# zdebruine/singlet

Measured on AMD Instinct MI355X. Metric: ALS iterations/sec (1M cells x 30k genes, 5% nnz, k=50), higher is better.
Workload: dtype f64

## Files before the change

### singlet_amd/csrc/kernels_dense.hip

```cpp
#include "sgl_internal.h"

typedef double d4 __attribute__((ext_vector_type(4)));

template <int NT>
__global__ __launch_bounds__(256) void gram_mfma_kernel(const double* __restrict__ F, int k, int64_t cols,
                                                        int64_t cols_per_block, double* __restrict__ part) {
    constexpr int NTILES = NT * (NT + 1) / 2;
    const int lane = threadIdx.x & 63, wave = threadIdx.x >> 6;
    const int r16 = lane & 15, kk = lane >> 4;
    const int64_t c_begin = (int64_t)blockIdx.x * cols_per_block;
    int64_t c_end = c_begin + cols_per_block;
    if (c_end > cols) c_end = cols;

    d4 acc[NTILES];
#pragma unroll
    for (int t = 0; t < NTILES; ++t) acc[t] = d4{0, 0, 0, 0};

    for (int64_t c = c_begin + 4 * wave; c < c_end; c += 16) {
        const int64_t cc = c + kk;
        double f[NT];
#pragma unroll
        for (int b = 0; b < NT; ++b) {
            const int row = b * 16 + r16;
            f[b] = (cc < c_end && row < k) ? F[cc * k + row] : 0.0;
        }
        int t = 0;
#pragma unroll
        for (int bi = 0; bi < NT; ++bi)
#pragma unroll
            for (int bj = 0; bj <= bi; ++bj) {
                acc[t] = __builtin_amdgcn_mfma_f64_16x16x4f64(f[bi], f[bj], acc[t], 0, 0, 0);
                ++t;
            }
    }

    __shared__ double sm[4][64 * 4];
    double* out = part + (size_t)blockIdx.x * k * k;
    int t = 0;
#pragma unroll
    for (int bi = 0; bi < NT; ++bi)
#pragma unroll
        for (int bj = 0; bj <= bi; ++bj) {
            __syncthreads();
#pragma unroll
            for (int r = 0; r < 4; ++r) sm[wave][lane * 4 + r] = acc[t][r];
            __syncthreads();
            if (wave == 0) {
#pragma unroll
                for (int r = 0; r < 4; ++r) {
                    const double v = ((sm[0][lane * 4 + r] + sm[1][lane * 4 + r]) + sm[2][lane * 4 + r]) + sm[3][lane * 4 + r];
                    const int row = bi * 16 + kk + 4 * r;
                    const int col = bj * 16 + r16;
                    if (row < k && col < k) {
                        out[(size_t)col * k + row] = v;
                        if (bi != bj) out[(size_t)row * k + col] = v;
                    }
                }
// ... 153 lines not shown
        for (int q = 0; q < nseg; ++q) s += tmp[q * n + t];
        out[t] = s + add_all;
    }
}
static size_t sgl_partial_ws(int nblocks, int n) { return (size_t)nblocks * n + (size_t)((nblocks + SGL_RED_SEG - 1) / SGL_RED_SEG) * n; }
static int sgl_partial_sum(sgl_ctx* c, int nblocks, int n, int diag_k, double diag_add, double* out, double add_all = 0.0) {
    const int nseg = (nblocks + SGL_RED_SEG - 1) / SGL_RED_SEG;
    if (diag_k == 0 && n * nseg <= 1024) {
        partial_sum_small_kernel<<<dim3(1), dim3(1024), 0, c->stream>>>(c->ws, nblocks, n, nseg, add_all, out);
        HIPCHK(hipGetLastError());
        return SGL_OK;
    }
    if (add_all != 0.0) { sgl_set_error("partial sum: add_all only in the short form"); return SGL_EINVAL; }
    double* tmp = c->ws + (size_t)nblocks * n;
    partial_sum_stage1_kernel<<<dim3((n + 255) / 256, nseg), dim3(256), 0, c->stream>>>(c->ws, nblocks, n, tmp);
    HIPCHK(hipGetLastError());
    partial_sum_stage2_kernel<<<dim3((n + 255) / 256), dim3(256), 0, c->stream>>>(tmp, nseg, n, diag_k, diag_add, out);
    HIPCHK(hipGetLastError());
    return SGL_OK;
}

int k_gram_big_partials(hipStream_t s, const double* F, int k, int64_t cols, int64_t cols_per_block, int nblocks, double* part);

int k_gram(sgl_ctx* c, const double* F, int k, int64_t cols, double* G, double diag_add) {
    if (k <= 0 || k > SGL_MAX_K) { sgl_set_error("k_gram: k=%d out of range", k); return SGL_EINVAL; }
    int nblocks = (int)((cols + 255) / 256);
    if (nblocks > 1024) nblocks = 1024;
    const bool big_mfma = k > 128 && k <= 256 && !getenv("SGL_GRAM_BIG_VALU");
    if (k > 128 && nblocks > (big_mfma ? 512 : 128)) nblocks = big_mfma ? 512 : 128;
    if (nblocks < 1) nblocks = 1;
    int64_t cpb = (cols + nblocks - 1) / nblocks;
    cpb = (cpb + 15) / 16 * 16;
    nblocks = (int)((cols + cpb - 1) / cpb);
    if (nblocks < 1) nblocks = 1;
    SGLCHK(sgl_ws_reserve(c, sizeof(double) * sgl_partial_ws(nblocks, k * k)));
    hipStream_t s = c->stream;
    const int NT = (k + 15) / 16;
    if (NT == 1) gram_mfma_kernel<1><<<dim3(nblocks), dim3(256), 0, s>>>(F, k, cols, cpb, c->ws);
    else if (NT == 2) gram_mfma_kernel<2><<<dim3(nblocks), dim3(256), 0, s>>>(F, k, cols, cpb, c->ws);
    else if (NT == 3) gram_mfma_kernel<3><<<dim3(nblocks), dim3(256), 0, s>>>(F, k, cols, cpb, c->ws);
    else if (NT == 4) gram_mfma_kernel<4><<<dim3(nblocks), dim3(256), 0, s>>>(F, k, cols, cpb, c->ws);
    else if (NT == 5) gram_mfma_split_kernel<5><<<dim3(nblocks), dim3(256), 0, s>>>(F, k, cols, cpb, c->ws);
    else if (NT == 6) gram_mfma_split_kernel<6><<<dim3(nblocks), dim3(256), 0, s>>>(F, k, cols, cpb, c->ws);
    else if (NT == 7) gram_mfma_split_kernel<7><<<dim3(nblocks), dim3(256), 0, s>>>(F, k, cols, cpb, c->ws);
    else if (NT == 8) gram_mfma_split_kernel<8><<<dim3(nblocks), dim3(256), 0, s>>>(F, k, cols, cpb, c->ws);
    else if (big_mfma) SGLCHK(k_gram_big_partials(s, F, k, cols, cpb, nblocks, c->ws));
    else {
        const size_t lds = sizeof(double) * 16 * (size_t)k;
        if (lds > 48 * 1024) HIPCHK(hipFuncSetAttribute(reinterpret_cast<const void*>(&gram_valu_kernel), hipFuncAttributeMaxDynamicSharedMemorySize, 144 * 1024));
        for (int pair0 = 0; pair0 < k * k; pair0 += 256 * GV_MAXP)
            gram_valu_kernel<<<dim3(nblocks), dim3(256), lds, s>>>(F, k, cols, cpb, c->ws, pair0);
    }
    HIPCHK(hipGetLastError());
    return sgl_partial_sum(c, nblocks, k * k, k, diag_add, G);
}

__global__ void add_diag_kernel(double* __restrict__ G, int k, double v) {
    const int i = blockIdx.x * blockDim.x + threadIdx.x;
    if (i < k) G[(size_t)i * k + i] += v;
}

int k_gram_add_diag(hipStream_t s, double* G, int k, double v) {
    add_diag_kernel<<<dim3((k + 63) / 64), dim3(64), 0, s>>>(G, k, v);
    HIPCHK(hipGetLastError());
    return SGL_OK;
}

__global__ __launch_bounds__(256) void rowsum_kernel(const double* __restrict__ F, int k, int64_t cols,
                                                     int64_t cols_per_block, double* __restrict__ part) {
    const int tx = threadIdx.x & 63, ty = threadIdx.x >> 6;
    const int64_t c_begin = (int64_t)blockIdx.x * cols_per_block;
    int64_t c_end = c_begin + cols_per_block;
    if (c_end > cols) c_end = cols;
    __shared__ double sm[4][64];
    for (int r0 = 0; r0 < k; r0 += 64) {
        const int row = r0 + tx;
        double s0 = 0.0, s1 = 0.0;
        if (row < k) {
            int64_t cc = c_begin + ty;
            for (; cc + 28 < c_end; cc += 32) {
                double v[8];
#pragma unroll
                for (int u = 0; u < 8; ++u) v[u] = F[(cc + 4 * u) * k + row];
#pragma unroll
                for (int u = 0; u < 8; u += 2) { s0 += v[u]; s1 += v[u + 1]; }
            }
            for (; cc + 4 < c_end; cc += 8) {
                s0 += F[cc * k + row];
                s1 += F[(cc + 4) * k + row];
            }
            if (cc < c_end) s0 += F[cc * k + row];
        }
        __syncthreads();
        sm[ty][tx] = s0 + s1;
        __syncthreads();
        if (ty == 0 && row < k) part[(size_t)blockIdx.x * k + row] = ((sm[0][tx] + sm[1][tx]) + sm[2][tx]) + sm[3][tx];
    }
}


int k_rowsum(sgl_ctx* c, const double* F, int k, int64_t cols, double* d_out, int add_eps) {
    int nblocks = (int)((cols + 511) / 512);
// ... 4 lines not shown
    rowsum_kernel<<<dim3(nblocks), dim3(256), 0, c->stream>>>(F, k, cols, cpb, c->ws);
    HIPCHK(hipGetLastError());
    const int nseg = (nblocks + SGL_RED_SEG - 1) / SGL_RED_SEG;
    if (add_eps && k * nseg > 1024) { sgl_set_error("k_rowsum: add_eps needs the short form"); return SGL_EINVAL; }
    return sgl_partial_sum(c, nblocks, k, 0, 0.0, d_out, add_eps ? 1e-15 : 0.0);
}
bool k_rowsum_can_add_eps(int k, int64_t cols) {
    int nblocks = (int)((cols + 511) / 512);
    if (nblocks > 512) nblocks = 512;
    if (nblocks < 1) nblocks = 1;
    return k * ((nblocks + SGL_RED_SEG - 1) / SGL_RED_SEG) <= 1024;
}

__global__ void add_eps_kernel(double* __restrict__ d, int k) {
    const int i = blockIdx.x * blockDim.x + threadIdx.x;
    if (i < k) d[i] += 1e-15;
}

__global__ void scale_kernel(double* __restrict__ F, int k, int64_t n, const double* __restrict__ d) {
    for (int64_t t = (int64_t)blockIdx.x * blockDim.x + threadIdx.x; t < n; t += (int64_t)gridDim.x * blockDim.x)
        F[t] = F[t] / d[t % k];
}

int k_scale_apply(hipStream_t s, double* F, int k, int64_t cols, double* d, int add_eps) {
    if (add_eps) {
        add_eps_kernel<<<dim3((k + 63) / 64), dim3(64), 0, s>>>(d, k);
        HIPCHK(hipGetLastError());
    }
    const int64_t n = (int64_t)k * cols;
    if (n <= 0) return SGL_OK;
    int64_t blocks = (n + 255) / 256;
    if (blocks > 4096) blocks = 4096;
    scale_kernel<<<dim3((unsigned)blocks), dim3(256), 0, s>>>(F, k, n, d);
    HIPCHK(hipGetLastError());
    return SGL_OK;
}

__global__ __launch_bounds__(256) void cor_partial_kernel(const double* __restrict__ x, const double* __restrict__ y,
                                                          int64_t n, double* __restrict__ part) {
    double s[5] = {0, 0, 0, 0, 0};
    for (int64_t t = (int64_t)blockIdx.x * blockDim.x + threadIdx.x; t < n; t += (int64_t)gridDim.x * blockDim.x) {
        const double a = x[t], b = y[t];
        s[0] += a;
        s[1] += b;
        s[2] = fma(a, b, s[2]);
        s[3] = fma(a, a, s[3]);
        s[4] = fma(b, b, s[4]);
    }
    __shared__ double sm[5][256];
    for (int q = 0; q < 5; ++q) sm[q][threadIdx.x] = s[q];
    __syncthreads();
// ... 123 lines not shown
```

### singlet_amd/csrc/multi.hip

```cpp
#include "sgl_internal.h"

#include <dlfcn.h>
#include <rccl/rccl.h>
#include <string.h>
#include <stdlib.h>
#include <algorithm>
#include <atomic>
#include <chrono>
#include <condition_variable>
#include <memory>
#include <functional>
#include <mutex>
#include <string>
#include <thread>
#include <vector>

struct RcclApi {
    void* handle = nullptr;
    char path[512] = "";
    ncclResult_t (*GetUniqueId)(ncclUniqueId*) = nullptr;
    ncclResult_t (*CommInitRank)(ncclComm_t*, int, ncclUniqueId, int) = nullptr;
    ncclResult_t (*CommInitAll)(ncclComm_t*, int, const int*) = nullptr;
    ncclResult_t (*CommDestroy)(ncclComm_t) = nullptr;
    ncclResult_t (*CommAbort)(ncclComm_t) = nullptr;
// ... 589 lines not shown
    auto halo_solve = [&](int i) -> int {
        sgl_ctx* c = T->local[i];
        SGLCHK(sgl_step_h_solve(c, L1_h, L2_h, true));
        Phase ph(c, SGL_PH_RHS_W);
        return k_graph_pack(c->stream, c->graph, c->H, k, T->rank[i]);
    };
    auto halo_partials = [&](int i) -> int {
        sgl_ctx* c = T->local[i];
        { Phase ph(c, SGL_PH_RHS_W); SGLCHK(k_graph_conv(c->stream, c->graph, c->H, c->B, k)); }
        SGLCHK(partials(c, c->B));
        book(i);
        return SGL_OK;
    };
    auto exchange1 = [&](int who) -> int {
        return team_exchange(T, who, {{1, &red, (int64_t)k * mb, false}, {0, &tail, (int64_t)k * k + k, false}});
    };
    auto gene_block = [&](int i) -> int {
        sgl_ctx* c = T->local[i];
        const int r = T->rank[i];
        double* Gh = c->red + (size_t)k * mpad;
        double* sh = Gh + (size_t)k * k;
        { Phase ph(c, SGL_PH_SCALE);
          HIPCHK(hipMemcpyAsync(c->d, sh, sizeof(double) * k, hipMemcpyDeviceToDevice, c->stream));
          SGLCHK(k_scale_apply(c->stream, c->H, k, c->A.ncol, c->d, 1)); }
        const int64_t g0 = (int64_t)r * mb;
        const int64_t ng = std::max<int64_t>(0, std::min<int64_t>(mb, m - g0));
        { Phase ph(c, SGL_PH_GRAM);
          HIPCHK(hipMemcpyAsync(c->G, Gh, sizeof(double) * k * k, hipMemcpyDeviceToDevice, c->stream));
          SGLCHK(k_gram_rescale(c->stream, c->G, k, c->d, 1e-15)); }
        Phase ph(c, SGL_PH_NNLS_W);
        if (ng > 0) {
            double* Bblk = c->red + (size_t)g0 * k;
            SGLCHK(k_scale_apply(c->stream, Bblk, k, ng, c->d, 0));
            if (c->link_w) SGLCHK(k_link_mul(c->stream, Bblk, c->link_w + (size_t)g0 * c->link_w_rows, k, c->link_w_rows, ng));
            else if (c->glink_w.table) SGLCHK(k_link_mul_grouped(c->stream, Bblk, c->glink_w.table, c->glink_w.group + g0, k, c->glink_w.rows, c->glink_w.groups, ng));
            const int64_t* gene_nnz = (N > 1) ? c->col_nnz_At_global : c->col_nnz_At;
            if (N > 1 && !c->gene_nnz_global) { sgl_set_error("team: global gene counts missing"); return SGL_ESTATE; }
            SGLCHK(sgl_nnls_shared(c, c->G, Bblk, c->W + (size_t)g0 * k, (c->solve_empty || graph) ? nullptr : gene_nnz + g0, ng, L1_w, L2_w, c->sweep_counters + 1));
        }
        return SGL_OK;
    };
    auto exchange2 = [&](int who) -> int {
        if (N <= 1) return SGL_OK;
        return team_exchange(T, who, {{2, &wbuf, (int64_t)k * mb, false}});
    };
    auto tail_part = [&](int i) -> int { return sgl_scale_w_enqueue(T->local[i]); };
// ... 35 lines not shown
    const int N = T->nranks;
    const int k = T->local[0]->k;
    const int64_t m = T->nrow;
    const int64_t mb = N > 1 ? (m + N - 1) / N : m;
    const int64_t mpad = mb * N;
    std::vector<void*> dv(nl), red(nl), sb(nl), tail(nl), wbuf(nl);
    std::vector<double> tols(nl, 0.0);
    auto h_update = [&](int i) -> int {
        sgl_ctx* c = T->local[i];
        SGLCHK(sgl_step_begin(c));
        SGLCHK(sgl_predict_mask_dev(c, c->A, c->col_nnz_A, c->W, c->H, c->B, seed, inv_density, L1, L2, 0, SGL_PH_RHS_H,
                                    SGL_PH_NNLS_H, c->sweep_counters + 0));
        Phase ph(c, SGL_PH_SCALE);
        SGLCHK(k_rowsum(c, c->H, k, c->A.ncol, c->d));
        dv[i] = c->d;
        return SGL_OK;
    };
    auto exchange_d = [&](int who) -> int {
        if (N <= 1) return SGL_OK;
        return team_exchange(T, who, {{0, &dv, (int64_t)k, false}});
    };
    auto w_partials = [&](int i) -> int {
        sgl_ctx* c = T->local[i];
        { Phase ph(c, SGL_PH_SCALE); SGLCHK(k_scale_apply(c->stream, c->H, k, c->A.ncol, c->d, 1)); }
        if (N == 1) {
            const int64_t* gene_nnz = c->col_nnz_At;
            return sgl_predict_mask_dev(c, c->At, gene_nnz, c->H, c->W, c->red, seed, inv_density, L1, L2, 1, SGL_PH_RHS_W,
                                        SGL_PH_NNLS_W, c->sweep_counters + 1);
        }
        double* Bw = c->red;
        double* Gh = c->red + (size_t)k * mpad;
        { Phase ph(c, SGL_PH_GRAM); SGLCHK(k_gram(c, c->H, k, c->A.ncol, Gh, 0.0)); }
        { Phase ph(c, SGL_PH_RHS_W); SGLCHK(sgl_masked_rhs(c, 1, c->H, Bw, seed, inv_density)); }
        { Phase ph(c, SGL_PH_MASK);
          HIPCHK(hipMemsetAsync(c->Sbuf, 0, sizeof(double) * (size_t)mpad * k * k, c->stream));
          if (!c->gene_nnz_global) { sgl_set_error("team: global gene counts missing"); return SGL_ESTATE; }
          const DevMaskList* ML = nullptr;
          if (k <= 128 && !getenv("SGL_MASK_NO_LIST")) {
              SGLCHK(sgl_mask_list_select(c, 1, m, c->At.nrow, seed, inv_density, 1, 0, c->cell_offset));
              if (c->ML[1].mask_t == 1) ML = &c->ML[1];
          }
          SGLCHK(k_mask_gram_cols(c->stream, 0, m, c->At.nrow, c->col_nnz_At_global, c->H, nullptr, k, seed, inv_density, 1, 0,
                                  c->cell_offset, c->Sbuf, ML)); }
        red[i] = Bw;
        if (c->Stri) {
            Phase ph(c, SGL_PH_MASK);
// ... 530 lines not shown
```

### singlet_amd/csrc/sgl_internal.h

```cpp
#pragma once
#include <hip/hip_runtime.h>
#include <stdint.h>
#include <stdio.h>
#include <stdarg.h>
#include <atomic>
#include <functional>
#include <vector>
#include <algorithm>

#include "../../include/singlet_hip.h"

#define SGL_WAVE 64
#define SGL_MAX_K 1024
#define SGL_LANE_NNLS_MAX_K 128

void sgl_set_error(const char* fmt, ...);

hipError_t sgl_pool_malloc_raw(void** p, size_t bytes);
template <typename T_>
inline hipError_t sgl_pool_malloc(T_** p, size_t bytes) { return sgl_pool_malloc_raw(reinterpret_cast<void**>(p), bytes); }
hipError_t sgl_pool_free(void* p);
hipError_t sgl_pool_mem_info(size_t* free_b, size_t* total_b);
void sgl_pool_release(void);
size_t sgl_pool_cached_bytes(void);
// ... 143 lines not shown
    int32_t* group = nullptr;
    int rows = 0, groups = 0;
};

struct sgl_ctx {
    int device = 0;
    hipStream_t own_stream = nullptr;
    hipStream_t stream = nullptr;

    DevCSC A, At;
    DevTiled TA, TAt;
    bool use_tiled = false;
    int64_t cell_offset = 0, ncells_total = 0;
    int64_t* col_nnz_A = nullptr;
    int64_t* col_nnz_At = nullptr;
    int64_t* col_nnz_At_global = nullptr;
    bool gene_nnz_global = false;

    int k = 0;
    double *W = nullptr, *Wprev = nullptr, *H = nullptr, *d = nullptr;
    double* B = nullptr;
    double* red = nullptr;
    double* G = nullptr;
    double* Gpad = nullptr;
    NnlsScratch nnls_scr;
    bool solve_empty = false;
    double* Adense = nullptr;
    bool dense_gemm = false;
    void* rocblas = nullptr;
    double* link_h = nullptr;
    double* link_w = nullptr;
    int link_h_rows = 0, link_w_rows = 0;
    DevGroupLink glink_h, glink_w;
    DevGraph graph;
    bool dense_input = false;
    DevMaskList ML[2];
    int64_t ml_builds[2] = {0, 0};
    DevMaskList MLkeep[2][SGL_ML_KEEP];
    double* Gcols = nullptr;
    int64_t gcols_chunk = 0;
    double* Wd = nullptr;
    double* Sbuf = nullptr;
    double* Stri = nullptr;
    struct sgl_team* team = nullptr;
    int team_rank = 0;
    double* ws = nullptr;
    size_t ws_bytes = 0;
    double* scalars = nullptr;
    unsigned long long* sweep_counters = nullptr;
    int64_t sweeps_acc[4] = {0, 0, 0, 0};
    int64_t wave_sweeps_acc[2] = {0, 0};
    double* pinned = nullptr;
    int64_t knn_last[4] = {0, 0, 0, 0};
    int64_t markers_last[4] = {0, 0, 0, 0};
    int64_t gsea_last[5] = {0, 0, 0, 0, 0};

    sgl_allreduce_fn allreduce = nullptr;
    void* allreduce_user = nullptr;

    bool timing = false;
    std::vector<PhaseEvent> pending;
    std::vector<hipEvent_t> event_pool;
    double phase_ms[SGL_PH_COUNT] = {0};
    int64_t phase_calls[SGL_PH_COUNT] = {0};
};

int sgl_team_size(const sgl_ctx* c);
int sgl_nnls_shared(sgl_ctx* c, const double* G, double* B, double* X, const int64_t* col_nnz, int64_t ncols,
                    double L1, double L2, unsigned long long* counter, bool h_side = false);
int sgl_step_h_rhs(sgl_ctx* c, bool convolve);
int sgl_step_h_solve(sgl_ctx* c, double L1, double L2, bool convolve);
int sgl_graph_check(const char* who, const double* Gx, const int32_t* Gi, const int32_t* Gp, int32_t G_nrow, int32_t G_ncol, int64_t n);
int sgl_graph_upload(sgl_ctx* c, const char* who, const double* Gx, const int32_t* Gi, const int32_t* Gp, int32_t ncol);
void sgl_graph_clear(sgl_ctx* c);
inline bool sgl_has_links(const sgl_ctx* c) { return c->link_h || c->link_w || c->glink_h.table || c->glink_w.table; }
int sgl_scale_w_enqueue(sgl_ctx* c);
int sgl_scale_w_fetch(sgl_ctx* c, double* tol);
int sgl_mask_workspace(sgl_ctx* c);
int sgl_predict_mask_dev(sgl_ctx* c, const DevCSC& M, const int64_t* col_nnz, const double* F, double* X, double* Bbuf,
                         uint64_t seed, uint64_t inv_density, double L1, double L2, int mask_t, int rhs_phase, int nnls_phase,
                         unsigned long long* counter);
int sgl_mse_test_enqueue(sgl_ctx* c, uint64_t seed, uint64_t inv_density);
#define SGL_MASK_MAX_K SGL_MAX_K
void sgl_team_detach(sgl_ctx* c);

int sgl_phase_begin(sgl_ctx* c, int phase, PhaseEvent* pe);
int sgl_phase_end(sgl_ctx* c, PhaseEvent* pe);
int sgl_ws_reserve(sgl_ctx* c, size_t bytes);
// ... 59 lines not shown
                     const sgl_callbacks* cb);

int k_rand(hipStream_t s, uint64_t state, const uint64_t* i, const uint64_t* j, int64_t n, uint64_t* out);
int k_mask(hipStream_t s, uint64_t state, uint64_t inv_density, int64_t cell0, int32_t ncells, int32_t ngenes, uint8_t* out);
int k_synth_count(hipStream_t s, uint64_t S, uint64_t inv_density, int transposed, int64_t cell_offset,
                  int32_t ncells, int32_t ngenes, int64_t* counts, const double* skew_dev = nullptr);
int k_synth_fill(hipStream_t s, uint64_t S, uint64_t inv_density, const double* levels16_dev, int transposed,
                 int64_t cell_offset, int32_t ncells, int32_t ngenes, const int64_t* p, int32_t* idx, double* x,
                 const double* skew_dev = nullptr);
int k_synth_winit(hipStream_t s, uint64_t S, int k, int32_t ngenes, double* W);
int k_exclusive_scan(sgl_ctx* c, const int64_t* in, int64_t* out, int64_t n);
int k_scan_total(hipStream_t s, const int64_t* in, int64_t* out, int64_t n);
int k_col_counts(hipStream_t s, const int64_t* p, int64_t ncol, int64_t* counts);
int k_validate_csc(hipStream_t s, const int32_t* idx, const int64_t* p, int64_t ncol, int32_t nrow, int* flag_dev);
int k_all_finite(hipStream_t s, const double* x, int64_t n, int* flag_dev);
int k_widen_p(hipStream_t s, const int32_t* p32, int64_t n1, int64_t* p64);
int k_build_segments(hipStream_t s, const DevCSC& M);

int k_gram(sgl_ctx* c, const double* F, int k, int64_t cols, double* G, double diag_add);
int k_gram_add_diag(hipStream_t s, double* G, int k, double v);
int k_rowsum(sgl_ctx* c, const double* F, int k, int64_t cols, double* d_out, int add_eps = 0);
bool k_rowsum_can_add_eps(int k, int64_t cols);
int k_scale_apply(hipStream_t s, double* F, int k, int64_t cols, double* d, int add_eps);
int k_cor(sgl_ctx* c, const double* x, const double* y, int64_t n, double* out_dev);
int k_pad_gram(hipStream_t s, const double* G, int k, int KP, int GS, double* Gpad);
int k_gram_rescale(hipStream_t s, double* G, int k, const double* d, double diag_add);
int k_i64_to_f64(hipStream_t s, const int64_t* in, double* out, int64_t n);
int k_f64_to_i64(hipStream_t s, const double* in, int64_t* out, int64_t n);
int k_transpose_dense(hipStream_t s, const double* in, int rows, int cols, double* out);

int k_acc(hipStream_t s, const DevCSC& M, const double* F, int k, double* B,
          uint64_t mask_seed, uint64_t inv_density, int mask_mode, int64_t mask_col_offset, int64_t mask_row_offset);

void sgl_tiled_free(DevTiled& S);
int sgl_tiled_build(sgl_ctx* c, const DevCSC& M, int k, DevTiled& S);
int k_acc_tiled(hipStream_t s, const DevTiled& S, const double* F, int ldf, double* B, int ldb, int kf, const double* xvals = nullptr);
int k_acc_tiled_all(hipStream_t s, const DevTiled& S, const double* F, double* B, int k, const double* xvals = nullptr);
int sgl_tiled_mask_values(sgl_ctx* c, const DevCSC& M, DevTiled& S, uint64_t seed, uint64_t inv_density, int mask_t,
                          int64_t col_off, int64_t row_off);
int sgl_masked_rhs(sgl_ctx* c, int orientation, const double* F, double* Bbuf, uint64_t seed, uint64_t inv_density);
int tiled_part_size(int k);

int k_dense_count(hipStream_t s, const double* A, int32_t nrow, int64_t ncol, int64_t* counts);
int k_dense_fill(hipStream_t s, const double* A, int32_t nrow, int64_t ncol, const int64_t* p, int32_t* idx, double* x);
int k_dense_rhs(sgl_ctx* c, int which, const double* F, int k, double* B);
void sgl_dense_release(sgl_ctx* c);
// ... 159 lines not shown
```

### singlet_amd/csrc/singlet_hip.hip

```cpp
#include "sgl_internal.h"
#include "ingest_host.h"

#include <math.h>
#include <string.h>
#include <algorithm>
#include <string>
#include <chrono>
#include <mutex>
#include <vector>
#include <stdlib.h>

static thread_local char g_err[1024] = "";

void sgl_set_error(const char* fmt, ...) {
    va_list ap;
    va_start(ap, fmt);
    vsnprintf(g_err, sizeof(g_err), fmt, ap);
    va_end(ap);
}

extern "C" const char* sgl_last_error(void) { return g_err; }
extern "C" int sgl_abi_version(void) { return 2; }

struct CallTimes {
// ... 117 lines not shown
    g = DevGraph();
}
void sgl_graph_clear(sgl_ctx* c) { free_graph(c); }

static void links_clear(sgl_ctx* c) {
    dev_free(c->link_h);
    dev_free(c->link_w);
    c->link_h_rows = c->link_w_rows = 0;
    for (DevGroupLink* g : {&c->glink_h, &c->glink_w}) {
        dev_free(g->table);
        dev_free(g->group);
        *g = DevGroupLink();
    }
}

static void free_fit(sgl_ctx* c, bool keep_streams = false) {
    dev_free(c->W);
    dev_free(c->Wprev);
    dev_free(c->H);
    dev_free(c->d);
    dev_free(c->B);
    dev_free(c->red);
    dev_free(c->G);
    dev_free(c->Gpad);
    dev_free(c->Gcols);
    c->gcols_chunk = 0;
    dev_free(c->Wd);
    dev_free(c->Sbuf);
    dev_free(c->Stri);
    nnls_scratch_free(c->nnls_scr);
    links_clear(c);
    free_graph(c);
    dev_free(c->A.seg);
    dev_free(c->At.seg);
    if (!keep_streams) {
        sgl_tiled_free(c->TA);
        sgl_tiled_free(c->TAt);
        sgl_mask_lists_free_all(c);
    }
    c->use_tiled = false;
    c->k = 0;
}

static void free_matrix(sgl_ctx* c) {
    sgl_dense_release(c);
    free_csc(c->A);
// ... 764 lines not shown
    if (rc == SGL_OK) rc = sgl_weight_by_split(c, split_by, n_groups);
    if (rc == SGL_OK) rc = sgl_download_csc(c, 0, x_out, nullptr, nullptr);
    sgl_destroy(c);
    return rc;
}

static int64_t team_gene_block(const sgl_ctx* c) {
    const int64_t m = c->A.nrow;
    const int n = sgl_team_size(c);
    return n > 1 ? (m + n - 1) / n : m;
}

static int fit_init_impl(sgl_ctx* c, int32_t k, const double* w_init, uint64_t synth_seed) {
    const int64_t m = c->A.nrow, n = c->A.ncol;
    const int64_t mpad = team_gene_block(c) * std::max(1, sgl_team_size(c));
    sgl_trace_setup(nullptr);
    SGLCHK(dev_alloc(&c->W, (size_t)k * mpad + 2));
    SGLCHK(dev_alloc(&c->Wprev, (size_t)k * m));
    SGLCHK(dev_alloc(&c->H, (size_t)k * n + 2));
    SGLCHK(dev_alloc(&c->d, (size_t)k));
    SGLCHK(dev_alloc(&c->B, (size_t)k * n + 2));
    SGLCHK(dev_alloc(&c->red, (size_t)k * mpad + (size_t)k * k + (size_t)k));
    SGLCHK(dev_alloc(&c->G, (size_t)k * k));
    SGLCHK(dev_alloc(&c->Gpad, (size_t)SGL_LANE_NNLS_MAX_K * (SGL_LANE_NNLS_MAX_K + 16) + 64));
    {
        const int64_t cap = std::max<int64_t>(c->A.ncol, c->A.nrow);
        if (k <= SGL_LANE_NNLS_MAX_K) SGLCHK(nnls_scratch_alloc(c->nnls_scr, cap, k));
        if (k <= 256 && c->A.ncol >= 65536) SGLCHK(nnls_pack_alloc(c->nnls_scr, c->A.ncol));
    }
    sgl_trace_setup("fit: factor buffers allocated");
    HIPCHK(hipMemsetAsync(c->W, 0, sizeof(double) * ((size_t)k * mpad + 2), c->stream));
    HIPCHK(hipMemsetAsync(c->red, 0, sizeof(double) * ((size_t)k * mpad + (size_t)k * k + (size_t)k), c->stream));
    if (w_init) HIPCHK(hipMemcpyAsync(c->W, w_init, sizeof(double) * (size_t)k * m, hipMemcpyHostToDevice, c->stream));
    else SGLCHK(k_synth_winit(c->stream, synth_seed, k, (int32_t)m, c->W));
    HIPCHK(hipMemsetAsync(c->H, 0, sizeof(double) * (size_t)k * n, c->stream));
    std::vector<double> ones((size_t)k, 1.0);
    HIPCHK(hipMemcpyAsync(c->d, ones.data(), sizeof(double) * k, hipMemcpyHostToDevice, c->stream));
    HIPCHK(hipStreamSynchronize(c->stream));
    sgl_trace_setup("fit: factors initialised");
    SGLCHK(build_tiles(c, c->A, k));
    SGLCHK(build_tiles(c, c->At, k));
    sgl_trace_setup("fit: build_tiles");
    c->use_tiled = false;
    if (tiled_part_size(k) > 0 && !getenv("SGL_NO_TILED")) {
        SGLCHK(sgl_tiled_build(c, c->A, tiled_part_size(k), c->TA));
        sgl_trace_setup("fit: entry stream of A done");
// ... 84 lines not shown
extern "C" int sgl_step_begin(sgl_ctx* c) {
    FIT_GUARD(c);
    Phase ph(c, SGL_PH_SCALE);
    HIPCHK(hipMemcpyAsync(c->Wprev, c->W, sizeof(double) * (size_t)c->k * c->A.nrow, hipMemcpyDeviceToDevice, c->stream));
    return SGL_OK;
}

int sgl_step_h_rhs(sgl_ctx* c, bool convolve) {
    const int k = c->k;
    { Phase ph(c, SGL_PH_GRAM); SGLCHK(k_gram(c, c->W, k, c->A.nrow, c->G, 1e-15)); }
    { Phase ph(c, SGL_PH_RHS_H);
      if (c->dense_gemm) SGLCHK(k_dense_rhs(c, 0, c->W, k, c->B));
      else if (c->use_tiled) SGLCHK(k_acc_tiled_all(c->stream, c->TA, c->W, c->B, k));
      else SGLCHK(k_acc(c->stream, c->A, c->W, k, c->B, 0, 1, 0, 0, 0));
      if (c->link_h) SGLCHK(k_link_mul(c->stream, c->B, c->link_h, k, c->link_h_rows, c->A.ncol));
      else if (c->glink_h.table) SGLCHK(k_link_mul_grouped(c->stream, c->B, c->glink_h.table, c->glink_h.group, k, c->glink_h.rows, c->glink_h.groups, c->A.ncol));
      if (c->graph.n && convolve) SGLCHK(k_graph_conv(c->stream, c->graph, c->B, c->graph.buf, k)); }
    return SGL_OK;
}

int sgl_step_h_solve(sgl_ctx* c, double L1, double L2, bool convolve) {
    const int k = c->k;
    if (c->graph.n && convolve) { Phase ph(c, SGL_PH_RHS_H); SGLCHK(k_graph_conv(c->stream, c->graph, c->B, c->graph.buf, k)); }
    { Phase ph(c, SGL_PH_NNLS_H);
      if (c->graph.n) SGLCHK(sgl_nnls_shared(c, c->G, c->graph.buf, c->H, nullptr, c->A.ncol, L1, L2, c->sweep_counters + 0, true));
      else SGLCHK(sgl_nnls_shared(c, c->G, c->B, c->H, c->solve_empty ? nullptr : c->col_nnz_A, c->A.ncol, L1, L2, c->sweep_counters + 0, true)); }
    return SGL_OK;
}

extern "C" int sgl_step_h(sgl_ctx* c, double L1, double L2) {
    FIT_GUARD(c);
    SGLCHK(sgl_step_h_rhs(c, true));
    return sgl_step_h_solve(c, L1, L2, false);
}

extern "C" int sgl_step_scale_h(sgl_ctx* c) {
    FIT_GUARD(c);
    if (c->team && sgl_team_size(c) > 1) { sgl_set_error("step API on a native team: use sgl_nmf_iterate / sgl_multi_iterate"); return SGL_ESTATE; }
    const int eps_in_sum = (!c->allreduce && k_rowsum_can_add_eps(c->k, c->A.ncol)) ? 1 : 0;
    { Phase ph(c, SGL_PH_SCALE); SGLCHK(k_rowsum(c, c->H, c->k, c->A.ncol, c->d, eps_in_sum)); }
    SGLCHK(do_allreduce(c, c->d, c->k));
    { Phase ph(c, SGL_PH_SCALE); SGLCHK(k_scale_apply(c->stream, c->H, c->k, c->A.ncol, c->d, eps_in_sum ? 0 : 1)); }
    return SGL_OK;
}

extern "C" int sgl_step_w(sgl_ctx* c, double L1, double L2) {
    FIT_GUARD(c);
    if (c->team && sgl_team_size(c) > 1) { sgl_set_error("step API on a native team: use sgl_nmf_iterate / sgl_multi_iterate"); return SGL_ESTATE; }
    const int k = c->k;
    const int64_t m = c->A.nrow;
    double* Bw = c->red;
    double* Gh = c->red + (size_t)k * m;
    const int64_t* gene_nnz = nullptr;
    SGLCHK(gene_counts(c, &gene_nnz));
    { Phase ph(c, SGL_PH_RHS_W);
      const double* F = c->H;
      if (c->graph.n) { SGLCHK(k_graph_conv(c->stream, c->graph, c->H, c->B, k)); F = c->B; }
      if (c->dense_gemm) SGLCHK(k_dense_rhs(c, 1, F, k, Bw));
      else if (c->use_tiled && c->TAt.roff) SGLCHK(k_acc_tiled_all(c->stream, c->TAt, F, Bw, k));
      else SGLCHK(k_acc(c->stream, c->At, F, k, Bw, 0, 1, 0, 0, 0)); }
    { Phase ph(c, SGL_PH_GRAM); SGLCHK(k_gram(c, c->H, k, c->A.ncol, Gh, 0.0)); }
    SGLCHK(do_allreduce(c, c->red, (int64_t)k * m + (int64_t)k * k));
    { Phase ph(c, SGL_PH_GRAM);
      HIPCHK(hipMemcpyAsync(c->G, Gh, sizeof(double) * k * k, hipMemcpyDeviceToDevice, c->stream));
      SGLCHK(k_gram_add_diag(c->stream, c->G, k, 1e-15)); }
    { Phase ph(c, SGL_PH_NNLS_W);
      if (c->link_w) SGLCHK(k_link_mul(c->stream, Bw, c->link_w, k, c->link_w_rows, m));
      else if (c->glink_w.table) SGLCHK(k_link_mul_grouped(c->stream, Bw, c->glink_w.table, c->glink_w.group, k, c->glink_w.rows, c->glink_w.groups, m));
      SGLCHK(sgl_nnls_shared(c, c->G, Bw, c->W, (c->solve_empty || c->graph.n) ? nullptr : gene_nnz, m, L1, L2, c->sweep_counters + 1)); }
    return SGL_OK;
}

int sgl_scale_w_enqueue(sgl_ctx* c) {
    const int k = c->k;
    const int64_t m = c->A.nrow;
    Phase ph(c, SGL_PH_SCALE);
    const int eps_in_sum = k_rowsum_can_add_eps(k, m) ? 1 : 0;
    SGLCHK(k_rowsum(c, c->W, k, m, c->d, eps_in_sum));
    SGLCHK(k_scale_apply(c->stream, c->W, k, m, c->d, eps_in_sum ? 0 : 1));
    SGLCHK(k_cor(c, c->W, c->Wprev, (int64_t)k * m, c->scalars));
    return SGL_OK;
}

int sgl_scale_w_fetch(sgl_ctx* c, double* tol_out) {
// ... 11 lines not shown

static int fetch_sweeps(sgl_ctx* c) {
    unsigned long long h[4] = {0, 0, 0, 0};
    HIPCHK(hipMemcpyAsync(h, c->sweep_counters, sizeof(h), hipMemcpyDeviceToHost, c->stream));
    HIPCHK(hipStreamSynchronize(c->stream));
    HIPCHK(hipMemsetAsync(c->sweep_counters, 0, sizeof(h), c->stream));
    c->sweeps_acc[0] += h[0];
    c->sweeps_acc[1] += h[1];
    c->wave_sweeps_acc[0] += h[2];
    c->wave_sweeps_acc[1] += h[3];
    return SGL_OK;
}

static bool interrupted(const sgl_callbacks* cb) {
    if (!(cb && cb->poll && cb->poll(cb->user))) return false;
    sgl_set_error("interrupted");
    return true;
}

int sgl_iterate_shard(sgl_ctx* c, double L1_w, double L1_h, double L2_w, double L2_h, const ArdArgs* mask, const sgl_callbacks* cb,
                      double* tol) {
    SGLCHK(sgl_step_begin(c));
    SGLCHK(mask ? sgl_step_h_masked(c, L1_h, L2_h, mask->seed, mask->inv_density) : sgl_step_h(c, L1_h, L2_h));
    SGLCHK(sgl_step_scale_h(c));
    if (interrupted(cb)) return SGL_EINTR;
    SGLCHK(mask ? sgl_step_w_masked(c, L1_w, L2_w, mask->seed, mask->inv_density) : sgl_step_w(c, L1_w, L2_w));
    return sgl_step_scale_w(c, tol);
}

int sgl_als_loop(double tol, int32_t maxit, const std::function<int(double*)>& iterate, const ArdArgs* ard,
                 const std::function<int(double*)>& mse_test, sgl_ctx* const* ctxs, int nctx, double* tol_trace, int32_t* n_iter,
                 const sgl_callbacks* cb) {
    double tol_ = 1.0;
    int it = 0, nt = 0;
    auto push_trace = [&](int iter_now) -> int {
        double err = 0.0;
        SGLCHK(mse_test(&err));
        ard->test_mse[nt] = err;
        ard->iter[nt] = iter_now;
        ard->tol_out[nt] = tol_;
        double min_err = ard->test_mse[0];
        for (int t = 1; t <= nt; ++t) min_err = std::min(min_err, ard->test_mse[t]);
        ard->score_overfit[nt] = (err - min_err) / (err + min_err);
        ++nt;
        return SGL_OK;
    };
    for (; it < maxit && tol_ > tol; ++it) {
// ... 9 lines not shown
        if (interrupted(cb)) return SGL_EINTR;
    }
    if (ard && it % ard->trace_test_mse != 0) SGLCHK(push_trace(it));
    for (int q = 0; q < nctx; ++q) {
        HIPCHK(hipSetDevice(ctxs[q]->device));
        SGLCHK(fetch_sweeps(ctxs[q]));
    }
    if (ard) *ard->n_trace = nt;
    if (n_iter) *n_iter = it;
    return SGL_OK;
}

extern "C" int sgl_nmf_run(sgl_ctx* c, double tol, int32_t maxit, double L1_w, double L1_h, double L2_w, double L2_h,
                           int32_t* n_iter, double* tol_trace, const sgl_callbacks* cb) {
    FIT_GUARD(c);
    auto iterate = [&](double* t) -> int {
        return c->team ? sgl_nmf_iterate(c, L1_w, L1_h, L2_w, L2_h, t) : sgl_iterate_shard(c, L1_w, L1_h, L2_w, L2_h, nullptr, cb, t);
    };
    return sgl_als_loop(tol, maxit, iterate, nullptr, nullptr, &c, 1, tol_trace, n_iter, cb);
}

extern "C" int sgl_project_run(sgl_ctx* c, double L1, double L2) {
    FIT_GUARD(c);
    HIPCHK(hipMemsetAsync(c->H, 0, sizeof(double) * (size_t)c->k * c->A.ncol, c->stream));
    SGLCHK(sgl_step_h(c, L1, L2));
    SGLCHK(sgl_step_scale_h(c));
    HIPCHK(hipStreamSynchronize(c->stream));
    return SGL_OK;
}

extern "C" int sgl_get_factors(sgl_ctx* c, double* w, double* d, double* h) {
    FIT_GUARD(c);
    HIPCHK(hipStreamSynchronize(c->stream));
    if (w) HIPCHK(hipMemcpy(w, c->W, sizeof(double) * (size_t)c->k * c->A.nrow, hipMemcpyDeviceToHost));
    if (d) HIPCHK(hipMemcpy(d, c->d, sizeof(double) * (size_t)c->k, hipMemcpyDeviceToHost));
    if (h) HIPCHK(hipMemcpy(h, c->H, sizeof(double) * (size_t)c->k * c->A.ncol, hipMemcpyDeviceToHost));
    return SGL_OK;
}

extern "C" int sgl_set_factors(sgl_ctx* c, const double* w, const double* d, const double* h) {
    FIT_GUARD(c);
    HIPCHK(hipStreamSynchronize(c->stream));
    if (w) HIPCHK(hipMemcpy(c->W, w, sizeof(double) * (size_t)c->k * c->A.nrow, hipMemcpyHostToDevice));
    if (d) HIPCHK(hipMemcpy(c->d, d, sizeof(double) * (size_t)c->k, hipMemcpyHostToDevice));
    if (h) HIPCHK(hipMemcpy(c->H, h, sizeof(double) * (size_t)c->k * c->A.ncol, hipMemcpyHostToDevice));
    return SGL_OK;
}

int sgl_mask_workspace(sgl_ctx* c) {
    const int k = c->k;
    if (!c->Gcols) {
        const int64_t widest = std::max<int64_t>(c->A.ncol, c->At.ncol);
        size_t free_b = 0, total_b = 0;
        HIPCHK(sgl_pool_mem_info(&free_b, &total_b));
        const char* e = getenv("SGL_GCOLS_MB");
        const int64_t mb = (e && atoll(e) > 0) ? atoll(e) : std::min<int64_t>(16384, std::max<int64_t>(256, (int64_t)(free_b >> 23)));
        const int64_t chunk = std::max<int64_t>(256, std::min<int64_t>(widest, (mb << 20) / ((int64_t)k * k * 8)));
        int rc = dev_alloc(&c->Gcols, (size_t)chunk * k * k);
        if (rc == SGL_ENOMEM && sgl_mask_lists_release_kept(c)) rc = dev_alloc(&c->Gcols, (size_t)chunk * k * k);
        SGLCHK(rc);
        c->gcols_chunk = chunk;
    }
    if (!c->Wd) SGLCHK(dev_alloc(&c->Wd, (size_t)k * c->A.nrow));
    return SGL_OK;
}

int sgl_masked_rhs(sgl_ctx* c, int orientation, const double* F, double* Bbuf, uint64_t seed, uint64_t inv_density) {
    const int mask_t = orientation ? 1 : 0;
    const DevCSC& M = orientation ? c->At : c->A;
    DevTiled& S = orientation ? c->TAt : c->TA;
    const int64_t col_off = mask_t ? 0 : c->cell_offset;
    const int64_t row_off = mask_t ? c->cell_offset : 0;
    if (c->use_tiled && S.roff && !getenv("SGL_MASKED_RHS_PLAIN")) {
        SGLCHK(sgl_tiled_mask_values(c, M, S, seed, inv_density, mask_t, col_off, row_off));
        return k_acc_tiled_all(c->stream, S, F, Bbuf, c->k, S.xm);
    }
    return k_acc(c->stream, M, F, c->k, Bbuf, seed, inv_density, mask_t ? 2 : 1, col_off, row_off);
}

int sgl_predict_mask_dev(sgl_ctx* c, const DevCSC& M, const int64_t* col_nnz, const double* F, double* X,
                            double* Bbuf, uint64_t seed, uint64_t inv_density, double L1, double L2, int mask_t,
                            int rhs_phase, int nnls_phase, unsigned long long* counter) {
    const int k = c->k;
    SGLCHK(sgl_mask_workspace(c));
    const int64_t col_off = mask_t ? 0 : c->cell_offset;
    const int64_t row_off = mask_t ? c->cell_offset : 0;
    { Phase ph(c, SGL_PH_GRAM); SGLCHK(k_gram(c, F, k, M.nrow, c->G, 1e-15)); }
    { Phase ph(c, rhs_phase);
      SGLCHK(sgl_masked_rhs(c, mask_t, F, Bbuf, seed, inv_density)); }
    const int64_t chunk = c->gcols_chunk;
    DevMaskList* L = nullptr;
    if (k <= 128 && !getenv("SGL_MASK_NO_LIST")) {
        Phase ph(c, SGL_PH_MASK);
        DevMaskList& Lm = c->ML[mask_t ? 1 : 0];
        SGLCHK(sgl_mask_list_select(c, mask_t ? 1 : 0, M.ncol, M.nrow, seed, inv_density, mask_t, col_off, row_off));
        if (Lm.mask_t == mask_t) L = &Lm;
    }
    for (int64_t c0 = 0; c0 < M.ncol; c0 += chunk) {
        const int64_t nc = std::min<int64_t>(chunk, M.ncol - c0);
        { Phase ph(c, SGL_PH_MASK);
          SGLCHK(k_mask_gram_cols(c->stream, c0, nc, M.nrow, col_nnz, F, c->G, k, seed, inv_density, mask_t, col_off, row_off, c->Gcols, L)); }
        { Phase ph(c, nnls_phase);
          SGLCHK(k_nnls_percol(c->stream, c->Gcols, (int64_t)k * k, Bbuf + (size_t)c0 * k, X + (size_t)c0 * k,
                             col_nnz ? col_nnz + c0 : nullptr, k, nc, L1, L2, counter)); }
    }
    return SGL_OK;
// ... 708 lines not shown
                          int32_t w_rows, int32_t w_cols, bool tr, double L1, double L2, bool scaled, double* h_out,
                          double* d_out) {
    const int k = tr ? w_cols : w_rows;
    const int64_t cols = tr ? w_rows : w_cols;
    if (cols != nrow) { sgl_set_error("'w' must share a common edge with the rows of 'A' (w is %d x %d, A has %d rows)", w_rows, w_cols, nrow); return SGL_EINVAL; }
    CtxHolder hd;
    SGLCHK(sgl_create(current_device_or_zero(), &hd.c));
    sgl_ctx* c = hd.c;
    SGLCHK(sgl_upload_csc_A_only(c, Ax, Ai, Ap, nrow, ncol));
    std::vector<double> wk;
    const double* wsrc = w;
    if (tr) {
        wk.resize((size_t)k * cols);
        for (int64_t r = 0; r < w_rows; ++r)
            for (int cidx = 0; cidx < w_cols; ++cidx) wk[(size_t)r * k + cidx] = w[(size_t)cidx * w_rows + r];
        wsrc = wk.data();
    }
    SGLCHK(sgl_fit_init(c, k, wsrc, 0));
    if (scaled) {
        SGLCHK(k_rowsum(c, c->W, k, nrow, c->d));
        SGLCHK(k_scale_apply(c->stream, c->W, k, nrow, c->d, 1));
        SGLCHK(sgl_project_run(c, L1, L2));
    } else {
        HIPCHK(hipMemsetAsync(c->H, 0, sizeof(double) * (size_t)k * ncol, c->stream));
        SGLCHK(sgl_step_h(c, L1, L2));
    }
    return sgl_get_factors(c, nullptr, d_out, h_out);
}

extern "C" int sgl_c_project_model(const double* Ax, const int32_t* Ai, const int32_t* Ap, int32_t nrow, int32_t ncol,
                                   const double* w, int32_t w_rows, int32_t w_cols, double L1, double L2,
                                   uint16_t threads, double* h_out, double* d_out) {
    (void)threads;
    if (!w || !h_out || !d_out) { sgl_set_error("sgl_c_project_model: NULL buffer"); return SGL_EINVAL; }
    return project_common(Ax, Ai, Ap, nrow, ncol, w, w_rows, w_cols, w_rows == nrow, L1, L2, true, h_out, d_out);
}

extern "C" int sgl_rcpp_predict(const double* Ax, const int32_t* Ai, const int32_t* Ap, int32_t nrow, int32_t ncol,
                                const double* w, int32_t w_rows, int32_t w_cols, double L1, double L2, uint16_t threads,
                                double* h_out) {
    (void)threads;
    if (!w || !h_out) { sgl_set_error("sgl_rcpp_predict: NULL buffer"); return SGL_EINVAL; }
    return project_common(Ax, Ai, Ap, nrow, ncol, w, w_rows, w_cols, w_rows == nrow && w_cols != nrow, L1, L2, false, h_out,
                          nullptr);
}

// ... 400 lines not shown
```

Before: 42.95.

## Fuse H scaling with H Gram computation and reuse cached Gram in W step

Measured after the change: 43.19 (median of 6 runs). About the same (+0.6%).

```diff
diff --git a/singlet_amd/csrc/kernels_dense.hip b/singlet_amd/csrc/kernels_dense.hip
--- a/singlet_amd/csrc/kernels_dense.hip
+++ b/singlet_amd/csrc/kernels_dense.hip
@@ -33,6 +33,98 @@
                 ++t;
             }
     }
+
+    __shared__ double sm[4][64 * 4];
+    double* out = part + (size_t)blockIdx.x * k * k;
+    int t = 0;
+#pragma unroll
+    for (int bi = 0; bi < NT; ++bi)
+#pragma unroll
+        for (int bj = 0; bj <= bi; ++bj) {
+            __syncthreads();
+#pragma unroll
+            for (int r = 0; r < 4; ++r) sm[wave][lane * 4 + r] = acc[t][r];
+            __syncthreads();
+            if (wave == 0) {
+#pragma unroll
+                for (int r = 0; r < 4; ++r) {
+                    const double v = ((sm[0][lane * 4 + r] + sm[1][lane * 4 + r]) + sm[2][lane * 4 + r]) + sm[3][lane * 4 + r];
+                    const int row = bi * 16 + kk + 4 * r;
+                    const int col = bj * 16 + r16;
+                    if (row < k && col < k) {
+                        out[(size_t)col * k + row] = v;
+                        if (bi != bj) out[(size_t)row * k + col] = v;
+                    }
+                }
+            }
+            ++t;
+        }
+}
+
+#ifndef SGL_SCALE_GRAM_PF
+#define SGL_SCALE_GRAM_PF 2
+#endif
+template <int NT, int PF>
+__global__ __launch_bounds__(256) void gram_scaled_mfma_kernel(double* __restrict__ F, int k, int64_t cols, int64_t cols_per_block,
+                                                               const double* __restrict__ d, double* __restrict__ part) {
+    constexpr int NTILES = NT * (NT + 1) / 2;
+    const int lane = threadIdx.x & 63;
+    const int wave = __builtin_amdgcn_readfirstlane((int)(threadIdx.x >> 6));
+    const int r16 = lane & 15, kk = lane >> 4;
+    const int64_t c_begin = (int64_t)blockIdx.x * cols_per_block;
+    int64_t c_end = c_begin + cols_per_block;
+    if (c_end > cols) c_end = cols;
+
+    d4 acc[NTILES];
+#pragma unroll
+    for (int t = 0; t < NTILES; ++t) acc[t] = d4{0, 0, 0, 0};
+
+    bool rok[NT];
+    double dr[NT];
+#pragma unroll
+    for (int b = 0; b < NT; ++b) {
+        rok[b] = b * 16 + r16 < k;
+        dr[b] = rok[b] ? d[b * 16 + r16] : 1.0;
+    }
+
+    int64_t c = c_begin + 4 * wave;
+    double* p = F + (c + kk) * k + r16;
+    const int64_t step = (int64_t)16 * k;
+    constexpr int R = PF + 1;
+    double raw[R][NT];
+    auto load_step = [&](double (&dst)[NT], const double* q, int64_t cq) {
+        const bool cok = cq + kk < c_end;
+#pragma unroll
+        for (int b = 0; b < NT; ++b) dst[b] = *((cok && rok[b]) ? q + b * 16 : d);
+    };
+#pragma unroll
+    for (int q = 0; q < PF; ++q) load_step(raw[q], p + q * step, c + 16 * q);
+    for (;;) {
+#pragma unroll
+        for (int q = 0; q < R; ++q) {
+            if (c >= c_end) goto steps_done;
+            load_step(raw[(q + PF) % R], p + PF * step, c + 16 * PF);
+            const bool cok = c + kk < c_end;
+            double f[NT];
+#pragma unroll
+            for (int b = 0; b < NT; ++b) {
+                const bool ok = cok && rok[b];
+                f[b] = ok ? raw[q][b] / dr[b] : 0.0;
+                if (ok) p[b * 16] = f[b];
+            }
+            int t = 0;
+#pragma unroll
+            for (int bi = 0; bi < NT; ++bi)
+#pragma unroll
+                for (int bj = 0; bj <= bi; ++bj) {
+                    acc[t] = __builtin_amdgcn_mfma_f64_16x16x4f64(f[bi], f[bj], acc[t], 0, 0, 0);
+                    ++t;
+                }
+            p += step;
+            c += 16;
+        }
+    }
+steps_done:
 
     __shared__ double sm[4][64 * 4];
     double* out = part + (size_t)blockIdx.x * k * k;
@@ -232,17 +324,43 @@
 
 int k_gram_big_partials(hipStream_t s, const double* F, int k, int64_t cols, int64_t cols_per_block, int nblocks, double* part);
 
-int k_gram(sgl_ctx* c, const double* F, int k, int64_t cols, double* G, double diag_add) {
-    if (k <= 0 || k > SGL_MAX_K) { sgl_set_error("k_gram: k=%d out of range", k); return SGL_EINVAL; }
+static void gram_blocks(int k, int64_t cols, bool big_mfma, int* nblocks_out, int64_t* cpb_out) {
     int nblocks = (int)((cols + 255) / 256);
     if (nblocks > 1024) nblocks = 1024;
-    const bool big_mfma = k > 128 && k <= 256 && !getenv("SGL_GRAM_BIG_VALU");
     if (k > 128 && nblocks > (big_mfma ? 512 : 128)) nblocks = big_mfma ? 512 : 128;
     if (nblocks < 1) nblocks = 1;
     int64_t cpb = (cols + nblocks - 1) / nblocks;
     cpb = (cpb + 15) / 16 * 16;
     nblocks = (int)((cols + cpb - 1) / cpb);
     if (nblocks < 1) nblocks = 1;
+    *nblocks_out = nblocks;
+    *cpb_out = cpb;
+}
+
+bool k_scale_gram_has(int k) { return k >= 1 && k <= 64; }
+int k_scale_gram(sgl_ctx* c, double* F, int k, int64_t cols, const double* d, double* G, double diag_add) {
+    if (!k_scale_gram_has(k)) { sgl_set_error("k_scale_gram: k=%d outside 1 .. 64", k); return SGL_EINVAL; }
+    if (cols <= 0) { sgl_set_error("k_scale_gram: no columns"); return SGL_EINVAL; }
+    int nblocks;
+    int64_t cpb;
+    gram_blocks(k, cols, false, &nblocks, &cpb);
+    SGLCHK(sgl_ws_reserve(c, sizeof(double) * sgl_partial_ws(nblocks, k * k)));
+    hipStream_t s = c->stream;
+    const int NT = (k + 15) / 16;
+    if (NT == 1) gram_scaled_mfma_kernel<1, SGL_SCALE_GRAM_PF><<<dim3(nblocks), dim3(256), 0, s>>>(F, k, cols, cpb, d, c->ws);
+    else if (NT == 2) gram_scaled_mfma_kernel<2, SGL_SCALE_GRAM_PF><<<dim3(nblocks), dim3(256), 0, s>>>(F, k, cols, cpb, d, c->ws);
+    else if (NT == 3) gram_scaled_mfma_kernel<3, SGL_SCALE_GRAM_PF><<<dim3(nblocks), dim3(256), 0, s>>>(F, k, cols, cpb, d, c->ws);
+    else gram_scaled_mfma_kernel<4, SGL_SCALE_GRAM_PF><<<dim3(nblocks), dim3(256), 0, s>>>(F, k, cols, cpb, d, c->ws);
+    HIPCHK(hipGetLastError());
+    return sgl_partial_sum(c, nblocks, k * k, k, diag_add, G);
+}
+
+int k_gram(sgl_ctx* c, const double* F, int k, int64_t cols, double* G, double diag_add) {
+    if (k <= 0 || k > SGL_MAX_K) { sgl_set_error("k_gram: k=%d out of range", k); return SGL_EINVAL; }
+    const bool big_mfma = k > 128 && k <= 256 && !getenv("SGL_GRAM_BIG_VALU");
+    int nblocks;
+    int64_t cpb;
+    gram_blocks(k, cols, big_mfma, &nblocks, &cpb);
     SGLCHK(sgl_ws_reserve(c, sizeof(double) * sgl_partial_ws(nblocks, k * k)));
     hipStream_t s = c->stream;
     const int NT = (k + 15) / 16;
@@ -278,7 +396,8 @@
 
 __global__ __launch_bounds__(256) void rowsum_kernel(const double* __restrict__ F, int k, int64_t cols,
                                                      int64_t cols_per_block, double* __restrict__ part) {
-    const int tx = threadIdx.x & 63, ty = threadIdx.x >> 6;
+    const int tx = threadIdx.x & 63;
+    const int ty = __builtin_amdgcn_readfirstlane((int)(threadIdx.x >> 6));
     const int64_t c_begin = (int64_t)blockIdx.x * cols_per_block;
     int64_t c_end = c_begin + cols_per_block;
     if (c_end > cols) c_end = cols;
@@ -288,6 +407,24 @@
         double s0 = 0.0, s1 = 0.0;
         if (row < k) {
             int64_t cc = c_begin + ty;
+            if (cc + 60 < c_end) {
+                double v[16], w[16];
+                auto load16 = [&](double (&dst)[16], int64_t c0) {
+#pragma unroll
+                    for (int u = 0; u < 16; ++u) dst[u] = F[(c0 + 4 * u) * k + row];
+                };
+                auto add16 = [&](const double (&src)[16]) {
+#pragma unroll
+                    for (int u = 0; u < 16; u += 2) { s0 += src[u]; s1 += src[u + 1]; }
+                };
+                load16(v, cc);
+                for (;;) {
+                    if (cc + 124 < c_end) { load16(w, cc + 64); add16(v); cc += 64; }
+                    else { add16(v); cc += 64; break; }
+                    if (cc + 124 < c_end) { load16(v, cc + 64); add16(w); cc += 64; }
+                    else { add16(w); cc += 64; break; }
+                }
+            }
             for (; cc + 28 < c_end; cc += 32) {
                 double v[8];
 #pragma unroll
@@ -338,11 +475,14 @@
         F[t] = F[t] / d[t % k];
 }
 
+int k_add_eps(hipStream_t s, double* d, int k) {
+    add_eps_kernel<<<dim3((k + 63) / 64), dim3(64), 0, s>>>(d, k);
+    HIPCHK(hipGetLastError());
+    return SGL_OK;
+}
+
 int k_scale_apply(hipStream_t s, double* F, int k, int64_t cols, double* d, int add_eps) {
-    if (add_eps) {
-        add_eps_kernel<<<dim3((k + 63) / 64), dim3(64), 0, s>>>(d, k);
-        HIPCHK(hipGetLastError());
-    }
+    if (add_eps) SGLCHK(k_add_eps(s, d, k));
     const int64_t n = (int64_t)k * cols;
     if (n <= 0) return SGL_OK;
     int64_t blocks = (n + 255) / 256;
diff --git a/singlet_amd/csrc/multi.hip b/singlet_amd/csrc/multi.hip
--- a/singlet_amd/csrc/multi.hip
+++ b/singlet_amd/csrc/multi.hip
@@ -635,6 +635,7 @@
         double* sh = Gh + (size_t)k * k;
         { Phase ph(c, SGL_PH_SCALE);
           HIPCHK(hipMemcpyAsync(c->d, sh, sizeof(double) * k, hipMemcpyDeviceToDevice, c->stream));
+          sgl_h_written(c);
           SGLCHK(k_scale_apply(c->stream, c->H, k, c->A.ncol, c->d, 1)); }
         const int64_t g0 = (int64_t)r * mb;
         const int64_t ng = std::max<int64_t>(0, std::min<int64_t>(mb, m - g0));
@@ -716,6 +717,7 @@
     };
     auto w_partials = [&](int i) -> int {
         sgl_ctx* c = T->local[i];
+        sgl_h_written(c);
         { Phase ph(c, SGL_PH_SCALE); SGLCHK(k_scale_apply(c->stream, c->H, k, c->A.ncol, c->d, 1)); }
         if (N == 1) {
             const int64_t* gene_nnz = c->col_nnz_At;
diff --git a/singlet_amd/csrc/sgl_internal.h b/singlet_amd/csrc/sgl_internal.h
--- a/singlet_amd/csrc/sgl_internal.h
+++ b/singlet_amd/csrc/sgl_internal.h
@@ -189,6 +189,8 @@
     double* B = nullptr;
     double* red = nullptr;
     double* G = nullptr;
+    double* Gh_kept = nullptr;
+    bool gram_h_valid = false;
     double* Gpad = nullptr;
     NnlsScratch nnls_scr;
     bool solve_empty = false;
@@ -231,6 +233,7 @@
     double phase_ms[SGL_PH_COUNT] = {0};
     int64_t phase_calls[SGL_PH_COUNT] = {0};
 };
+inline void sgl_h_written(sgl_ctx* c) { c->gram_h_valid = false; }
 
 int sgl_team_size(const sgl_ctx* c);
 int sgl_nnls_shared(sgl_ctx* c, const double* G, double* B, double* X, const int64_t* col_nnz, int64_t ncols,
@@ -336,6 +339,9 @@
 int k_rowsum(sgl_ctx* c, const double* F, int k, int64_t cols, double* d_out, int add_eps = 0);
 bool k_rowsum_can_add_eps(int k, int64_t cols);
 int k_scale_apply(hipStream_t s, double* F, int k, int64_t cols, double* d, int add_eps);
+int k_add_eps(hipStream_t s, double* d, int k);
+bool k_scale_gram_has(int k);
+int k_scale_gram(sgl_ctx* c, double* F, int k, int64_t cols, const double* d, double* G, double diag_add);
 int k_cor(sgl_ctx* c, const double* x, const double* y, int64_t n, double* out_dev);
 int k_pad_gram(hipStream_t s, const double* G, int k, int KP, int GS, double* Gpad);
 int k_gram_rescale(hipStream_t s, double* G, int k, const double* d, double diag_add);
diff --git a/singlet_amd/csrc/singlet_hip.hip b/singlet_amd/csrc/singlet_hip.hip
--- a/singlet_amd/csrc/singlet_hip.hip
+++ b/singlet_amd/csrc/singlet_hip.hip
@@ -163,6 +163,8 @@
     dev_free(c->B);
     dev_free(c->red);
     dev_free(c->G);
+    dev_free(c->Gh_kept);
+    sgl_h_written(c);
     dev_free(c->Gpad);
     dev_free(c->Gcols);
     c->gcols_chunk = 0;
@@ -973,6 +975,7 @@
     SGLCHK(dev_alloc(&c->B, (size_t)k * n + 2));
     SGLCHK(dev_alloc(&c->red, (size_t)k * mpad + (size_t)k * k + (size_t)k));
     SGLCHK(dev_alloc(&c->G, (size_t)k * k));
+    if (k_scale_gram_has(k)) SGLCHK(dev_alloc(&c->Gh_kept, (size_t)k * k));
     SGLCHK(dev_alloc(&c->Gpad, (size_t)SGL_LANE_NNLS_MAX_K * (SGL_LANE_NNLS_MAX_K + 16) + 64));
     {
         const int64_t cap = std::max<int64_t>(c->A.ncol, c->A.nrow);
@@ -1103,6 +1106,7 @@
 int sgl_step_h_solve(sgl_ctx* c, double L1, double L2, bool convolve) {
     const int k = c->k;
     if (c->graph.n && convolve) { Phase ph(c, SGL_PH_RHS_H); SGLCHK(k_graph_conv(c->stream, c->graph, c->B, c->graph.buf, k)); }
+    sgl_h_written(c);
     { Phase ph(c, SGL_PH_NNLS_H);
       if (c->graph.n) SGLCHK(sgl_nnls_shared(c, c->G, c->graph.buf, c->H, nullptr, c->A.ncol, L1, L2, c->sweep_counters + 0, true));
       else SGLCHK(sgl_nnls_shared(c, c->G, c->B, c->H, c->solve_empty ? nullptr : c->col_nnz_A, c->A.ncol, L1, L2, c->sweep_counters + 0, true)); }
@@ -1119,9 +1123,25 @@
     FIT_GUARD(c);
     if (c->team && sgl_team_size(c) > 1) { sgl_set_error("step API on a native team: use sgl_nmf_iterate / sgl_multi_iterate"); return SGL_ESTATE; }
     const int eps_in_sum = (!c->allreduce && k_rowsum_can_add_eps(c->k, c->A.ncol)) ? 1 : 0;
+    sgl_h_written(c);
     { Phase ph(c, SGL_PH_SCALE); SGLCHK(k_rowsum(c, c->H, c->k, c->A.ncol, c->d, eps_in_sum)); }
     SGLCHK(do_allreduce(c, c->d, c->k));
     { Phase ph(c, SGL_PH_SCALE); SGLCHK(k_scale_apply(c->stream, c->H, c->k, c->A.ncol, c->d, eps_in_sum ? 0 : 1)); }
+    return SGL_OK;
+}
+
+static bool scale_gram_fused(const sgl_ctx* c) {
+    return !c->team && !c->allreduce && c->Gh_kept != nullptr && k_scale_gram_has(c->k) && c->A.ncol > 0 && !getenv("SGL_NO_FUSED_SCALE_GRAM");
+}
+static int scale_h_fused(sgl_ctx* c) {
+    const int k = c->k;
+    const int eps_in_sum = k_rowsum_can_add_eps(k, c->A.ncol) ? 1 : 0;
+    sgl_h_written(c);
+    { Phase ph(c, SGL_PH_SCALE);
+      SGLCHK(k_rowsum(c, c->H, k, c->A.ncol, c->d, eps_in_sum));
+      if (!eps_in_sum) SGLCHK(k_add_eps(c->stream, c->d, k)); }
+    { Phase ph(c, SGL_PH_GRAM); SGLCHK(k_scale_gram(c, c->H, k, c->A.ncol, c->d, c->Gh_kept, 0.0)); }
+    c->gram_h_valid = true;
     return SGL_OK;
 }
 
@@ -1140,7 +1160,10 @@
       if (c->dense_gemm) SGLCHK(k_dense_rhs(c, 1, F, k, Bw));
       else if (c->use_tiled && c->TAt.roff) SGLCHK(k_acc_tiled_all(c->stream, c->TAt, F, Bw, k));
       else SGLCHK(k_acc(c->stream, c->At, F, k, Bw, 0, 1, 0, 0, 0)); }
-    { Phase ph(c, SGL_PH_GRAM); SGLCHK(k_gram(c, c->H, k, c->A.ncol, Gh, 0.0)); }
+    { Phase ph(c, SGL_PH_GRAM);
+      if (!(c->gram_h_valid && c->Gh_kept)) SGLCHK(k_gram(c, c->H, k, c->A.ncol, Gh, 0.0));
+      else if (c->allreduce) HIPCHK(hipMemcpyAsync(Gh, c->Gh_kept, sizeof(double) * k * k, hipMemcpyDeviceToDevice, c->stream));
+      else Gh = c->Gh_kept; }
     SGLCHK(do_allreduce(c, c->red, (int64_t)k * m + (int64_t)k * k));
     { Phase ph(c, SGL_PH_GRAM);
       HIPCHK(hipMemcpyAsync(c->G, Gh, sizeof(double) * k * k, hipMemcpyDeviceToDevice, c->stream));
@@ -1198,7 +1221,8 @@
                       double* tol) {
     SGLCHK(sgl_step_begin(c));
     SGLCHK(mask ? sgl_step_h_masked(c, L1_h, L2_h, mask->seed, mask->inv_density) : sgl_step_h(c, L1_h, L2_h));
-    SGLCHK(sgl_step_scale_h(c));
+    if (!mask && scale_gram_fused(c)) SGLCHK(scale_h_fused(c));
+    else SGLCHK(sgl_step_scale_h(c));
     if (interrupted(cb)) return SGL_EINTR;
     SGLCHK(mask ? sgl_step_w_masked(c, L1_w, L2_w, mask->seed, mask->inv_density) : sgl_step_w(c, L1_w, L2_w));
     return sgl_step_scale_w(c, tol);
@@ -1254,6 +1278,7 @@
 
 extern "C" int sgl_project_run(sgl_ctx* c, double L1, double L2) {
     FIT_GUARD(c);
+    sgl_h_written(c);
     HIPCHK(hipMemsetAsync(c->H, 0, sizeof(double) * (size_t)c->k * c->A.ncol, c->stream));
     SGLCHK(sgl_step_h(c, L1, L2));
     SGLCHK(sgl_step_scale_h(c));
@@ -1275,6 +1300,7 @@
     HIPCHK(hipStreamSynchronize(c->stream));
     if (w) HIPCHK(hipMemcpy(c->W, w, sizeof(double) * (size_t)c->k * c->A.nrow, hipMemcpyHostToDevice));
     if (d) HIPCHK(hipMemcpy(c->d, d, sizeof(double) * (size_t)c->k, hipMemcpyHostToDevice));
+    if (h) sgl_h_written(c);
     if (h) HIPCHK(hipMemcpy(c->H, h, sizeof(double) * (size_t)c->k * c->A.ncol, hipMemcpyHostToDevice));
     return SGL_OK;
 }
@@ -1314,6 +1340,7 @@
                             double* Bbuf, uint64_t seed, uint64_t inv_density, double L1, double L2, int mask_t,
                             int rhs_phase, int nnls_phase, unsigned long long* counter) {
     const int k = c->k;
+    if (X == c->H) sgl_h_written(c);
     SGLCHK(sgl_mask_workspace(c));
     const int64_t col_off = mask_t ? 0 : c->cell_offset;
     const int64_t row_off = mask_t ? c->cell_offset : 0;
@@ -2068,6 +2095,7 @@
         SGLCHK(k_scale_apply(c->stream, c->W, k, nrow, c->d, 1));
         SGLCHK(sgl_project_run(c, L1, L2));
     } else {
+        sgl_h_written(c);
         HIPCHK(hipMemsetAsync(c->H, 0, sizeof(double) * (size_t)k * ncol, c->stream));
         SGLCHK(sgl_step_h(c, L1, L2));
     }
```
